# sebastian-hofstaetter/matchmaker

Hardware: NVIDIA H100
Metric: query-doc pairs scored/sec (ColBERT max-sim d=128) (higher is better)
Workload: dtype f16

## Files before the change

matchmaker_b200/build.py:

```python
from __future__ import annotations

import argparse
import hashlib
import os
import shutil
import subprocess
import sys
from concurrent.futures import ThreadPoolExecutor

HERE = os.path.dirname(os.path.abspath(__file__))
CSRC = os.path.join(HERE, "csrc")
INCLUDE = os.path.join(os.path.dirname(HERE), "include")
LIB_NAME = "libmatchmaker_b200.so"
LIB_PATH = os.path.join(CSRC, LIB_NAME)
OBJ_DIR = os.path.join(CSRC, "build")

NVCC_FLAGS = [
    "-gencode", "arch=compute_90a,code=sm_90a",
    "-O3", "-std=c++17", "-lineinfo",
    "-Xcompiler", "-fPIC",
    "-Xcompiler", "-fvisibility=hidden",
    "--expt-relaxed-constexpr",
    "-I", INCLUDE,
]


def _nvcc() -> str:
    for cand in (os.environ.get("NVCC"), shutil.which("nvcc"), "/usr/local/cuda/bin/nvcc"):
        if cand and os.path.isfile(cand):
            return cand
    raise RuntimeError("nvcc not found (set NVCC=...)")


def sources():
    return sorted(os.path.join(CSRC, f) for f in os.listdir(CSRC) if f.endswith(".cu"))


def _digest(paths) -> str:
    h = hashlib.sha256()
    for p in sorted(paths):
        h.update(p.encode())
        with open(p, "rb") as f:
            h.update(f.read())
    h.update(" ".join(NVCC_FLAGS).encode())
    return h.hexdigest()


def _all_inputs():
    hdrs = [os.path.join(CSRC, f) for f in os.listdir(CSRC) if f.endswith((".cuh", ".h"))]
    hdrs += [os.path.join(INCLUDE, f) for f in os.listdir(INCLUDE) if f.endswith(".h")]
    return sources() + hdrs


def build(force: bool = False, verbose: bool = False, prof: bool = False) -> str:
    stamp = os.path.join(OBJ_DIR, "stamp.sha256")
    digest = _digest(_all_inputs()) + ("+prof" if prof else "")
    if not force and os.path.isfile(LIB_PATH) and os.path.isfile(stamp) and open(stamp).read() == digest:
        return LIB_PATH
    os.makedirs(OBJ_DIR, exist_ok=True)
    nvcc = _nvcc()
    extra = (["-Xptxas", "-v"] if verbose else []) + (["-DMMB200_ENABLE_PROF"] if prof else [])

    def compile_one(src):
        obj = os.path.join(OBJ_DIR, os.path.basename(src)[:-3] + ".o")
        cmd = [nvcc, *NVCC_FLAGS, *extra, "-c", src, "-o", obj]
        r = subprocess.run(cmd, capture_output=True, text=True)
        if r.returncode != 0:
            raise RuntimeError(f"nvcc failed for {src}:\n{r.stdout}\n{r.stderr}")
        if verbose:
            sys.stderr.write(r.stderr)
        return obj

    with ThreadPoolExecutor(max_workers=min(8, os.cpu_count() or 1)) as ex:
        objs = list(ex.map(compile_one, sources()))
    link = [nvcc, "-shared", "-gencode", "arch=compute_90a,code=sm_90a", "-cudart", "static",
            "-Xcompiler", "-fPIC", "-o", LIB_PATH, *objs]
    r = subprocess.run(link, capture_output=True, text=True)
    if r.returncode != 0:
        raise RuntimeError(f"link failed:\n{r.stdout}\n{r.stderr}")
    with open(stamp, "w") as f:
        f.write(digest)
    return LIB_PATH


if __name__ == "__main__":
    ap = argparse.ArgumentParser()
    ap.add_argument("--force", action="store_true")
    ap.add_argument("--verbose", action="store_true")
    ap.add_argument("--prof", action="store_true", help="debugging build with the MMB200_*_PROF switches compiled in")
    a = ap.parse_args()
    print(build(force=a.force, verbose=a.verbose, prof=a.prof))
```

matchmaker_b200/csrc/maxsim_qm.cu:

```cuda
#include <cuda_bf16.h>
#include <cuda_fp16.h>

#include <algorithm>

#include "device_util.cuh"
#include "host_util.cuh"
#include "masks.cuh"
#include "maxsim.cuh"
#include "ptx.cuh"

namespace mmb {

namespace {

constexpr int kThreads = 384;
constexpr int kChunkRows = 64;
constexpr int kChunkKBlockBytes = kChunkRows * 128;
constexpr int kMaxStages = 32;
constexpr int kMaxLd = 4096;
constexpr int kScouts = 3;
constexpr int kRecordStep = 6;
constexpr int kMaxRecords = 48;
constexpr int kRecordReserve = 12 * 1024;
constexpr int kQSlots = 2;
constexpr int kQRows = 32;
constexpr int kQBlockBytes = kQRows * 128;
constexpr uint32_t kFill = 1u << 16, kLiveMask = kFill - 1;
constexpr int kRecBits = 4;
constexpr int kRegsHelper = 120, kRegsConsumer = 192;

#ifdef MMB200_ENABLE_PROF
enum QmProf {
  kPrTotal, kPrQEmpty, kPrRFull, kPrEmpty, kPrTma, kPrChunks,
  kCoTotal, kCoRFull, kCoFull, kCoIssue, kCoMma, kCoReduce, kCoEpilogue, kCoDocs,
  kScTotal, kScREmpty,
  kProfCount
};
__device__ unsigned long long g_qm_prof[kProfCount];
#define QM_PROF(...) __VA_ARGS__
#else
#define QM_PROF(...)
#endif

struct QmShared {
  uint64_t full[kMaxStages];
  uint64_t empty[kMaxStages];
  uint64_t qfull[kQSlots];
  uint64_t qempty[kQSlots];
  uint64_t rfull[kMaxRecords];
  uint64_t rempty[kMaxRecords];
  float xm[2][2][4][32];
  int32_t xa[2][2][4][32];
};

struct QmLaunch {
  int32_t kblocks;
  int32_t stages;
  int32_t chunk_bytes;
  int32_t records;
  int32_t rec_words;
};

struct RecCursor {
  int slot;
  uint32_t phase;
  __device__ __forceinline__ void advance(int step, int records) {
    slot += step;
    if (slot >= records) { slot -= records; phase ^= 1u; }
  }
};

struct QmMaps {
  CUtensorMap q;
  CUtensorMap d;
};

template <bool kStore>
struct PairStream {
  struct Batch {
    int32_t q, d, dm, rows;
    int64_t row0, row_end;
  };
  const MaxsimParams& P;
  int64_t first, end, step;
  int64_t pre_batch;
  int k;
  int lane;
  Batch cur, nxt, pre;

  __device__ __forceinline__ PairStream(const MaxsimParams& P_, int64_t first_, int64_t end_, int64_t step_, int lane_)
      : P(P_), first(first_), end(end_), step(step_), lane(lane_) {
    load1(cur, 0);
    load1(nxt, 1);
    load2(cur);
    load2(nxt);
    resolve(cur);
    pre_batch = 2;
    load1(pre, pre_batch);
    k = -1;
  }
  __device__ __forceinline__ void load1(Batch& b, int64_t bi) {
    const int64_t p = first + (bi * 32 + lane) * step;
    b.q = 0; b.d = -1; b.dm = 0; b.rows = 0; b.row0 = 0; b.row_end = 0;
    if (p >= end) return;
    b.q = P.pair_q ? P.pair_q[p] : (int32_t)((p + P.pair_base) / P.docs_per_query);
    b.d = P.pair_d ? P.pair_d[p] : (int32_t)p;
    if (P.pair_dmask) b.dm = P.pair_dmask[p];
  }
  __device__ __forceinline__ void load2(Batch& b) {
    if (!P.pair_dmask) b.dm = b.d;
    if constexpr (kStore) {
      if (b.d >= 0) { b.row0 = P.doc_offsets[b.d]; b.row_end = P.doc_offsets[b.d + 1]; }
    }
  }
  __device__ __forceinline__ void resolve(Batch& b) {
    if constexpr (kStore) b.rows = (int)max((int64_t)0, min(b.row_end - b.row0, (int64_t)P.Ld));
  }
  __device__ __forceinline__ void next() {
    if (++k == 32) {
      cur = nxt;
      resolve(cur);
      nxt = pre;
      load2(nxt);
      load1(pre, ++pre_batch);
      k = 0;
    }
  }
  __device__ __forceinline__ int64_t q() const { return __shfl_sync(0xffffffffu, cur.q, k); }
  __device__ __forceinline__ int64_t d() const { return __shfl_sync(0xffffffffu, cur.d, k); }
  __device__ __forceinline__ int64_t dm() const { return __shfl_sync(0xffffffffu, cur.dm, k); }
  __device__ __forceinline__ int rows() const { return __shfl_sync(0xffffffffu, cur.rows, k); }
  __device__ __forceinline__ int64_t row0() const { return __shfl_sync(0xffffffffu, cur.row0, k); }
};

template <typename T>
__device__ __forceinline__ void wgmma_n32(float (&d)[16], uint64_t a, uint64_t b, uint32_t acc);
template <>
__device__ __forceinline__ void wgmma_n32<__half>(float (&d)[16], uint64_t a, uint64_t b, uint32_t acc) {
  wgmma_m64n32k16_f16(d, a, b, acc);
}
template <>
__device__ __forceinline__ void wgmma_n32<__nv_bfloat16>(float (&d)[16], uint64_t a, uint64_t b, uint32_t acc) {
  wgmma_m64n32k16_bf16(d, a, b, acc);
}

template <bool kArgmax>
__device__ __forceinline__ void take(float v, int row, float& m, int& am) {
  if constexpr (kArgmax) {
    const bool gt = v > m;
    m = gt ? v : m;
    am = gt ? row : am;
  } else {
    m = fmaxf(m, v);
  }
}

template <typename T, bool kArgmax, bool kStore>
__global__ void __launch_bounds__(kThreads, 1)
maxsim_qm_kernel(const __grid_constant__ QmMaps M, MaxsimParams P, QmLaunch L) {
  extern __shared__ uint8_t smem_raw[];
  uint8_t* smem = smem_raw + ((1024u - (smem_u32(smem_raw) & 1023u)) & 1023u);
  const int qslot_bytes = L.kblocks * kQBlockBytes;
  uint8_t* q_base = smem;
  uint8_t* stage_base = q_base + kQSlots * qslot_bytes;
  uint32_t* rec_base = reinterpret_cast<uint32_t*>(stage_base + (size_t)L.stages * L.chunk_bytes);
  QmShared* S = reinterpret_cast<QmShared*>(rec_base + (size_t)L.records * L.rec_words);

  const int warp = threadIdx.x >> 5;
  const int lane = threadIdx.x & 31;

  int64_t p_begin, p_end;
  cta_share(P.n_pairs, &p_begin, &p_end);

  if (threadIdx.x == 0) {
    prefetch_tensormap(&M.q);
    prefetch_tensormap(&M.d);
    for (int s = 0; s < L.stages; ++s) { mbar_init(&S->full[s], 1); mbar_init(&S->empty[s], 4); }
    for (int s = 0; s < kQSlots; ++s) { mbar_init(&S->qfull[s], 1); mbar_init(&S->qempty[s], 8); }
    for (int r = 0; r < L.records; ++r) {
      mbar_init(&S->rfull[r], 1);
      mbar_init(&S->rempty[r], 5);
      rec_base[(size_t)r * L.rec_words + kRecBits - 2] = 0;
      rec_base[(size_t)r * L.rec_words + kRecBits - 1] = 0;
    }
    fence_barrier_init();
  }
  __syncthreads();

  if (warp == 0) {
    setmaxnreg_dec<kRegsHelper>();
    PairStream<kStore> meta(P, p_begin, p_end, 1, lane);
    const int ring = L.stages >> 1;
    int st_cur = 0, st_oth = 0;
    uint32_t ph_cur = 0, ph_oth = 0;
    int64_t prev_q = -1;
    uint32_t qcount = 0;
    RecCursor rc{0, 0};
    QM_PROF(unsigned long long prof[kProfCount] = {}; const long long t_start = clock64(); long long t_;)
    for (int64_t p = p_begin; p < p_end; ++p) {
      meta.next();
      const int64_t qi = meta.q();
      const int64_t di = meta.d();
      const int64_t row0 = kStore ? meta.row0() : 0;
      if (qi != prev_q) {
        const uint32_t slot = qcount & 1u, use = qcount >> 1;
        QM_PROF(t_ = clock64();)
        mbar_wait(&S->qempty[slot], (use & 1u) ^ 1u);
        QM_PROF(prof[kPrQEmpty] += clock64() - t_;)
        if (elect_one_sync()) {
          mbar_arrive_expect_tx(&S->qfull[slot], (uint32_t)(L.kblocks * kQBlockBytes));
          for (int kb = 0; kb < L.kblocks; ++kb)
            tma_load_4d(&M.q, q_base + (size_t)slot * qslot_bytes + kb * kQBlockBytes, &S->qfull[slot], 0, 0, kb, (int)qi,
                        kEvictLast);
        }
        __syncwarp();
        ++qcount;
        prev_q = qi;
      }
      const int c = (int)((p - p_begin) & 1);
      QM_PROF(t_ = clock64();)
      mbar_wait(&S->rfull[rc.slot], rc.phase);
      QM_PROF(prof[kPrRFull] += clock64() - t_;)
      const int live = (int)(rec_base[(size_t)rc.slot * L.rec_words] & kLiveMask);
      __syncwarp();
      if (lane == 0) mbar_arrive(&S->rempty[rc.slot]);
      rc.advance(1, L.records);
      const int dcoord = kStore ? 0 : (int)di;
      const int nch = max(1, (live + kChunkRows - 1) / kChunkRows);
      int row = kStore ? (int)row0 : live - kChunkRows * nch;
      for (int ch = 0; ch < nch; ++ch, row += kChunkRows) {
        const int stage = c * ring + st_cur;
        QM_PROF(t_ = clock64();)
        mbar_wait(&S->empty[stage], ph_cur ^ 1u);
        QM_PROF(prof[kPrEmpty] += clock64() - t_; t_ = clock64(); ++prof[kPrChunks];)
        if (elect_one_sync()) {
          if (live == 0) {
            mbar_arrive(&S->full[stage]);
          } else {
            mbar_arrive_expect_tx(&S->full[stage], (uint32_t)L.chunk_bytes);
            tma_load_4d(&M.d, stage_base + (size_t)stage * L.chunk_bytes, &S->full[stage], 0, row, 0, dcoord, kEvictFirst);
          }
        }
        __syncwarp();
        QM_PROF(prof[kPrTma] += clock64() - t_;)
        if (++st_cur == ring) { st_cur = 0; ph_cur ^= 1u; }
      }
      const int st = st_cur; st_cur = st_oth; st_oth = st;
      const uint32_t ph = ph_cur; ph_cur = ph_oth; ph_oth = ph;
    }
    QM_PROF(prof[kPrTotal] = clock64() - t_start;
            if (lane == 0) for (int i = kPrTotal; i <= kPrChunks; ++i) atomicAdd(&g_qm_prof[i], prof[i]);)
  } else if (warp <= kScouts) {
    setmaxnreg_dec<kRegsHelper>();
    constexpr int kW = 8;
    const int s = warp - 1;
    const int dmt = P.d_mask ? P.mask_dtype : MMB200_MASK_NONE;
    const int nwin = (P.Ld + 32 * kW - 1) / (32 * kW);
    const int bit_words = L.rec_words - kRecBits;
    PairStream<kStore> meta(P, p_begin + s, p_end, kScouts, lane);
    RecCursor rc{s, 0};
    int64_t fp = p_begin + s;
    auto load_win = [&](uint32_t (&raw)[kW], int64_t dm, int w) {
#pragma unroll
      for (int k = 0; k < kW; ++k) {
        const int g = w * 32 * kW + 32 * k + lane;
        raw[k] = 1;
        if (dmt != MMB200_MASK_NONE && g < P.Ld) {
          const uint64_t v = mask_raw(P.d_mask, dmt, dm * (int64_t)P.Ld + g);
          raw[k] = (uint32_t)(v | (v >> 32));
        }
      }
    };
    auto fetch = [&](uint32_t (&raw)[kW], int64_t& dm, int& lim) {
      if (fp < p_end) {
        meta.next();
        dm = meta.dm();
        lim = kStore ? meta.rows() : P.Ld;
        load_win(raw, dm, 0);
      }
      fp += kScouts;
    };
    QM_PROF(unsigned long long prof_re = 0; const long long t_start = clock64();)
    auto doc = [&](uint32_t (&raw)[kW], int64_t& dm, int& lim) {
      QM_PROF(const long long t_ = clock64();)
      mbar_wait(&S->rempty[rc.slot], rc.phase ^ 1u);
      QM_PROF(prof_re += clock64() - t_;)
      uint32_t* rec = rec_base + (size_t)rc.slot * L.rec_words;
      int live = 0;
      bool masked = false;
      for (int w = 0; w < nwin; ++w) {
        if (w > 0) load_win(raw, dm, w);
#pragma unroll
        for (int k = 0; k < kW; ++k) {
          const int g = w * 32 * kW + 32 * k + lane;
          const bool in_doc = g < lim;
          const bool ok = in_doc && mask_test(raw[k], dmt);
          masked |= in_doc && !ok;
          const uint32_t b = __ballot_sync(0xffffffffu, ok);
          const int wi = w * kW + k;
          if (b) live = 32 * wi + 32 - __clz(b);
          if (lane == 0 && wi < bit_words) rec[kRecBits + wi] = b;
        }
      }
      const bool fill = !kStore && __any_sync(0xffffffffu, masked);
      fetch(raw, dm, lim);
      if (lane == 0) {
        rec[0] = (uint32_t)live | (fill ? kFill : 0u);
        mbar_arrive(&S->rfull[rc.slot]);
      }
      rc.advance(kScouts, L.records);
    };
    uint32_t ra[kW], rb[kW];
    int64_t dma = 0, dmb = 0;
    int la = 0, lb = 0;
    fetch(ra, dma, la);
    fetch(rb, dmb, lb);
    for (int64_t sp = p_begin + s; sp < p_end;) {
      doc(ra, dma, la);
      if ((sp += kScouts) >= p_end) break;
      doc(rb, dmb, lb);
      sp += kScouts;
    }
    QM_PROF(if (lane == 0) {
      atomicAdd(&g_qm_prof[kScTotal], (unsigned long long)(clock64() - t_start));
      atomicAdd(&g_qm_prof[kScREmpty], prof_re);
    })
  } else {
    setmaxnreg_inc<kRegsConsumer>();
    const int c = (warp >> 2) - 1;
    const int wq = warp & 3;
    const int r0 = 16 * wq + (lane >> 2);
    const int qmt = P.q_mask ? P.mask_dtype : MMB200_MASK_NONE;
    const int ring = L.stages >> 1;
    int64_t prev_q = -1;
    uint32_t qcount = 0;
    int cur_slot = 0;
    RecCursor rc{c, 0};
    auto load_q = [&](int64_t n0) -> int32_t { return p_begin + n0 + lane < p_end ? P.pair_q[p_begin + n0 + lane] : 0; };
    int32_t qb_cur = 0, qb_nxt = 0;
    if (P.pair_q) { qb_cur = load_q(0); qb_nxt = load_q(32); }
    int64_t q_run = 0;
    int32_t q_rem = 0;
    if (!P.pair_q) {
      q_run = (p_begin + P.pair_base) / P.docs_per_query;
      q_rem = (int32_t)((p_begin + P.pair_base) - q_run * P.docs_per_query);
    }
    QM_PROF(unsigned long long prof[kProfCount] = {}; const long long t_start = clock64(); long long t_;)
    int64_t n_walk = 0;
    auto walk_to = [&](int64_t n) {
      for (; n_walk <= n; ++n_walk) {
        int64_t qi;
        if (P.pair_q) {
          if ((n_walk & 31) == 0 && n_walk > 0) { qb_cur = qb_nxt; qb_nxt = load_q(n_walk + 32); }
          qi = __shfl_sync(0xffffffffu, qb_cur, (int)(n_walk & 31));
        } else {
          qi = q_run;
          if (++q_rem == P.docs_per_query) { q_rem = 0; ++q_run; }
        }
        if (qi != prev_q) {
          if (prev_q >= 0) { __syncwarp(); if (lane == 0) mbar_arrive(&S->qempty[cur_slot]); }
          cur_slot = (int)(qcount & 1u);
          mbar_wait(&S->qfull[cur_slot], (qcount >> 1) & 1u);
          ++qcount;
          prev_q = qi;
        }
      }
      return prev_q;
    };
    struct Doc {
      int64_t n;
      uint32_t qlo;
      uint64_t qraw;
      int slot;
      uint32_t head;
      int live, nch;
    };
    auto begin = [&](Doc& D, int64_t n) {
      const int64_t qi = walk_to(n);
      D.n = n;
      D.qlo = (uint32_t)make_wgmma_sw128_desc(smem_u32(q_base + (size_t)cur_slot * qslot_bytes));
      D.qraw = 0;
      if (wq == 0 && lane < P.Lq)
        D.qraw = (qmt != MMB200_MASK_NONE) ? mask_raw(P.q_mask, qmt, qi * (int64_t)P.Lq + lane) : 1;
      QM_PROF(t_ = clock64();)
      mbar_wait(&S->rfull[rc.slot], rc.phase);
      QM_PROF(prof[kCoRFull] += clock64() - t_; ++prof[kCoDocs];)
      D.slot = rc.slot;
      rc.advance(2, L.records);
      D.head = rec_base[(size_t)D.slot * L.rec_words];
      D.live = (int)(D.head & kLiveMask);
      D.nch = max(1, (D.live + kChunkRows - 1) / kChunkRows);
    };
    int st_next = 0;
    uint32_t ph_next = 0;
    constexpr uint64_t kDescHi = (uint64_t)(1024 >> 4) << 32 | (uint64_t)1 << 62;
    auto issue = [&](float (&acc)[16], uint32_t qlo_doc) -> int {
      const int stage = c * ring + st_next;
      QM_PROF(t_ = clock64();)
      mbar_wait(&S->full[stage], ph_next);
      QM_PROF(prof[kCoFull] += clock64() - t_; t_ = clock64();)
      if (++st_next == ring) { st_next = 0; ph_next ^= 1u; }
      const uint32_t daddr = smem_u32(stage_base + (size_t)stage * L.chunk_bytes);
      const uint32_t dlo = (uint32_t)make_wgmma_sw128_desc(__shfl_sync(0xffffffffu, daddr, 0));
      const uint32_t qlo = __shfl_sync(0xffffffffu, qlo_doc, 0);
      wgmma_fence();
#pragma unroll
      for (int k = 0; k < 4; ++k) wgmma_n32<T>(acc, kDescHi | (dlo + 2 * k), kDescHi | (qlo + 2 * k), k != 0);
      if (L.kblocks > 1) {
#pragma unroll
        for (int k = 0; k < 4; ++k)
          wgmma_n32<T>(acc, kDescHi | (dlo + (kChunkKBlockBytes >> 4) + 2 * k),
                       kDescHi | (qlo + (kQBlockBytes >> 4) + 2 * k), 1);
      }
      wgmma_commit();
      wgmma_fence_regs(acc);
      QM_PROF(prof[kCoIssue] += clock64() - t_;)
      return stage;
    };
    float mx[8];
    int ax[8];
#pragma unroll
    for (int e = 0; e < 8; ++e) { mx[e] = -INFINITY; ax[e] = -1; }
    auto reduce = [&](float (&acc)[16], int stage, const Doc& D, int ch) {
      wgmma_fence_regs(acc);
      const int col0 = kStore ? kChunkRows * ch : D.live - kChunkRows * (D.nch - ch);
      const int x0 = col0 + r0, x1 = x0 + 8;
      const uint32_t* bits = rec_base + (size_t)D.slot * L.rec_words + kRecBits;
      const float p0 = (bits[x0 >> 5] >> (x0 & 31)) & 1u ? 0.f : -INFINITY;
      const float p1 = (bits[x1 >> 5] >> (x1 & 31)) & 1u ? 0.f : -INFINITY;
#pragma unroll
      for (int e = 0; e < 8; ++e) {
        const int i = 4 * (e >> 1) + (e & 1);
        take<kArgmax>(acc[i] + p0, x0, mx[e], ax[e]);
        take<kArgmax>(acc[i + 2] + p1, x1, mx[e], ax[e]);
      }
      __syncwarp();
      if (lane == 0) mbar_arrive(&S->empty[stage]);
    };
    auto combine = [&](float om, int oa, float& m, int& a) {
      if constexpr (kArgmax) {
        if (om > m || (om == m && (unsigned)oa < (unsigned)a)) { m = om; a = oa; }
      } else {
        m = fmaxf(m, om);
      }
    };
    auto epilogue = [&](const Doc& D) {
      QM_PROF(t_ = clock64();)
      if (lane == 0) mbar_arrive(&S->rempty[D.slot]);
#pragma unroll
      for (int o = 4; o < 32; o <<= 1) {
#pragma unroll
        for (int e = 0; e < 8; ++e) {
          const float om = __shfl_xor_sync(0xffffffffu, mx[e], o);
          const int oa = kArgmax ? __shfl_xor_sync(0xffffffffu, ax[e], o) : 0;
          combine(om, oa, mx[e], ax[e]);
        }
      }
      const int buf = (int)((D.n >> 1) & 1);
      float* xm = S->xm[c][buf][0];
      int32_t* xa = S->xa[c][buf][0];
      if (lane < 4) {
#pragma unroll
        for (int e = 0; e < 8; ++e) {
          const int t = 8 * (e >> 1) + 2 * lane + (e & 1);
          xm[32 * wq + t] = mx[e];
          if constexpr (kArgmax) xa[32 * wq + t] = ax[e];
        }
      }
#pragma unroll
      for (int e = 0; e < 8; ++e) { mx[e] = -INFINITY; ax[e] = -1; }
      if (wq != 0) {
        named_bar_arrive(1 + c, 128);
      } else {
        named_bar_sync(1 + c, 128);
        float m = xm[lane];
        int a = kArgmax ? xa[lane] : -1;
#pragma unroll
        for (int w = 1; w < 4; ++w) combine(xm[32 * w + lane], kArgmax ? xa[32 * w + lane] : 0, m, a);
        if (D.head & kFill) take<kArgmax>(-1000.f, P.Ld, m, a);
        const bool ok = mask_test(D.qraw, qmt);
        const int64_t p = p_begin + D.n;
        if constexpr (kArgmax) {
          if (lane < P.Lq) P.argmax[p * (int64_t)P.Lq + lane] = (ok && a < P.Ld) ? a : -1;
        }
        float s = ok ? m : 0.f;
        s += __shfl_down_sync(0xffffffffu, s, 8);
#pragma unroll
        for (int o = 1; o < 8; o <<= 1) s += __shfl_xor_sync(0xffffffffu, s, o);
        const float hi = __shfl_sync(0xffffffffu, s, 16);
        if (lane == 0) P.out[p] = s + hi;
      }
      QM_PROF(prof[kCoEpilogue] += clock64() - t_;)
    };
    const int64_t n_pairs = p_end - p_begin;
    float acc[16];
    for (int64_t n = c; n < n_pairs; n += 2) {
      Doc D;
      begin(D, n);
      for (int ch = 0; ch < D.nch; ++ch) {
        const int st = issue(acc, D.qlo);
        QM_PROF(t_ = clock64();)
        wgmma_wait<0>();
        QM_PROF(prof[kCoMma] += clock64() - t_; t_ = clock64();)
        reduce(acc, st, D, ch);
        QM_PROF(prof[kCoReduce] += clock64() - t_;)
      }
      epilogue(D);
    }
    QM_PROF(prof[kCoTotal] = clock64() - t_start;
            if (wq == 0 && lane == 0) for (int i = kCoTotal; i <= kCoDocs; ++i) atomicAdd(&g_qm_prof[i], prof[i]);)
  }
}

template <typename T, bool kArgmax, bool kStore>
int launch_qm(int grid, size_t smem_bytes, cudaStream_t stream, const QmMaps& M, const MaxsimParams& P,
              const QmLaunch& L) {
  MMB_CHECK_CUDA(cudaFuncSetAttribute(maxsim_qm_kernel<T, kArgmax, kStore>, cudaFuncAttributeMaxDynamicSharedMemorySize,
                                      (int)smem_bytes));
  maxsim_qm_kernel<T, kArgmax, kStore><<<grid, kThreads, smem_bytes, stream>>>(M, P, L);
  MMB_CHECK_CUDA(cudaGetLastError());
  return MMB200_OK;
}

int launch_qm_dispatch(int grid, size_t smem_bytes, cudaStream_t stream, const QmMaps& M, const MaxsimParams& P,
                       const QmLaunch& L, int dtype) {
  if (P.doc_offsets)
    return dtype == MMB200_F16 ? launch_qm<__half, false, true>(grid, smem_bytes, stream, M, P, L)
                               : launch_qm<__nv_bfloat16, false, true>(grid, smem_bytes, stream, M, P, L);
  if (dtype == MMB200_F16)
    return P.argmax ? launch_qm<__half, true, false>(grid, smem_bytes, stream, M, P, L)
                    : launch_qm<__half, false, false>(grid, smem_bytes, stream, M, P, L);
  return P.argmax ? launch_qm<__nv_bfloat16, true, false>(grid, smem_bytes, stream, M, P, L)
                  : launch_qm<__nv_bfloat16, false, false>(grid, smem_bytes, stream, M, P, L);
}

}

int maxsim_qm_launch(const MaxsimParams& P, int dtype, const DeviceInfo& dev, cudaStream_t stream, bool* handled) {
  *handled = false;
  if (dtype != MMB200_F16 && dtype != MMB200_BF16) return MMB200_OK;
  if (P.Lq > kQRows || (P.dim != 64 && P.dim != 128) || P.Ld > kMaxLd) return MMB200_OK;
  if ((reinterpret_cast<uintptr_t>(P.q) | reinterpret_cast<uintptr_t>(P.d)) & 15) return MMB200_OK;
  if (P.doc_offsets && P.argmax) return MMB200_OK;
  QmLaunch L;
  L.kblocks = P.dim / 64;
  L.chunk_bytes = L.kblocks * kChunkKBlockBytes;
  L.rec_words = kRecBits + 2 * ((P.Ld + kChunkRows - 1) / kChunkRows);
  const int fixed = kQSlots * L.kblocks * kQBlockBytes + (int)sizeof(QmShared) + 1024;
  L.stages = std::min(kMaxStages, (dev.max_smem_optin - fixed - kRecordReserve) / L.chunk_bytes) & ~1;
  const int rec_bytes = L.rec_words * 4;
  L.records = std::min(kMaxRecords, (dev.max_smem_optin - fixed - L.stages * L.chunk_bytes) / rec_bytes);
  L.records -= L.records % kRecordStep;
  if (L.stages < 4 || L.records < kRecordStep) return MMB200_OK;
  const size_t smem_bytes = (size_t)L.stages * L.chunk_bytes + (size_t)L.records * rec_bytes + fixed;

  const CUtensorMapDataType tdt = dtype == MMB200_F16 ? CU_TENSOR_MAP_DATA_TYPE_FLOAT16 : CU_TENSOR_MAP_DATA_TYPE_BFLOAT16;
  QmMaps M;
  {
    const uint64_t dims[4] = {64, (uint64_t)P.Lq, (uint64_t)L.kblocks, (uint64_t)P.n_q};
    const uint64_t strides[3] = {(uint64_t)P.dim * 2, 128, (uint64_t)P.Lq * P.dim * 2};
    const uint32_t box[4] = {64, (uint32_t)kQRows, 1, 1};
    if (int rc = encode_tensor_map(&M.q, tdt, 4, P.q, dims, strides, box, CU_TENSOR_MAP_SWIZZLE_128B,
                                   CU_TENSOR_MAP_L2_PROMOTION_L2_128B))
      return rc;
  }
  const uint64_t d_rows = P.doc_offsets ? (uint64_t)P.n_rows : (uint64_t)P.Ld;
  const uint64_t d_count = P.doc_offsets ? 1 : (uint64_t)P.n_d;
  {
    const uint64_t dims[4] = {64, d_rows, (uint64_t)L.kblocks, d_count};
    const uint64_t strides[3] = {(uint64_t)P.dim * 2, 128, d_rows * P.dim * 2};
    const uint32_t box[4] = {64, (uint32_t)kChunkRows, (uint32_t)L.kblocks, 1};
    if (int rc = encode_tensor_map(&M.d, tdt, 4, P.d, dims, strides, box, CU_TENSOR_MAP_SWIZZLE_128B,
                                   CU_TENSOR_MAP_L2_PROMOTION_L2_256B))
      return rc;
  }
  *handled = true;
  const int grid = (int)std::min<int64_t>(dev.sm_count, P.n_pairs);
#ifdef MMB200_ENABLE_PROF
  const bool prof = getenv("MMB200_MAXSIM_PROF") != nullptr;
  if (prof) {
    const unsigned long long zero[kProfCount] = {};
    MMB_CHECK_CUDA(cudaMemcpyToSymbolAsync(g_qm_prof, zero, sizeof(zero), 0, cudaMemcpyHostToDevice, stream));
  }
  const int rc = launch_qm_dispatch(grid, smem_bytes, stream, M, P, L, dtype);
  if (prof && rc == MMB200_OK) {
    unsigned long long h[kProfCount];
    MMB_CHECK_CUDA(cudaMemcpyFromSymbolAsync(h, g_qm_prof, sizeof(h), 0, cudaMemcpyDeviceToHost, stream));
    MMB_CHECK_CUDA(cudaStreamSynchronize(stream));
    const double ctas = grid, wgs = 2.0 * grid, scouts = (double)kScouts * grid;
    const double chunks = (double)h[kPrChunks], docs = (double)h[kCoDocs];
    fprintf(stderr,
            "maxsim_prof pairs %lld Ld %d chunks %.0f | cycles per CTA: producer total %.0f qempty %.0f rfull %.0f "
            "empty %.0f tma %.0f | per consumer warpgroup: total %.0f rfull %.0f full %.0f issue %.0f mma %.0f "
            "reduce %.0f epilogue %.0f | per scout: total %.0f rempty %.0f | per chunk: producer %.0f (empty %.0f, "
            "tma %.0f), warpgroup full %.0f issue %.0f mma %.0f reduce %.0f | per document per warpgroup: total %.0f "
            "epilogue %.0f rfull %.0f\n",
            (long long)P.n_pairs, P.Ld, chunks, h[kPrTotal] / ctas, h[kPrQEmpty] / ctas, h[kPrRFull] / ctas,
            h[kPrEmpty] / ctas, h[kPrTma] / ctas, h[kCoTotal] / wgs, h[kCoRFull] / wgs, h[kCoFull] / wgs,
            h[kCoIssue] / wgs, h[kCoMma] / wgs, h[kCoReduce] / wgs, h[kCoEpilogue] / wgs, h[kScTotal] / scouts,
            h[kScREmpty] / scouts, h[kPrTotal] / chunks, h[kPrEmpty] / chunks, h[kPrTma] / chunks, h[kCoFull] / chunks,
            h[kCoIssue] / chunks, h[kCoMma] / chunks, h[kCoReduce] / chunks, h[kCoTotal] / docs, h[kCoEpilogue] / docs,
            h[kCoRFull] / docs);
  }
  return rc;
#else
  return launch_qm_dispatch(grid, smem_bytes, stream, M, P, L, dtype);
#endif
}

}
```

matchmaker_b200/csrc/ptx.cuh:

```cuda
#pragma once

#include <cuda.h>
#include <cuda_runtime.h>
#include <stdint.h>

namespace mmb {

__device__ __forceinline__ uint32_t smem_u32(const void* p) {
  return static_cast<uint32_t>(__cvta_generic_to_shared(p));
}

__device__ __forceinline__ uint32_t lane_id() { return threadIdx.x & 31u; }


__device__ __forceinline__ void mbar_init(uint64_t* bar, uint32_t count) {
  asm volatile("mbarrier.init.shared::cta.b64 [%0], %1;" ::"r"(smem_u32(bar)), "r"(count) : "memory");
}

__device__ __forceinline__ void fence_barrier_init() {
  asm volatile("fence.mbarrier_init.release.cluster;" ::: "memory");
}

__device__ __forceinline__ void fence_proxy_async_smem() {
  asm volatile("fence.proxy.async.shared::cta;" ::: "memory");
}

__device__ __forceinline__ void mbar_arrive(uint64_t* bar) {
  asm volatile("{\n\t.reg .b64 st;\n\tmbarrier.arrive.shared::cta.b64 st, [%0];\n\t}" ::"r"(smem_u32(bar))
               : "memory");
}

__device__ __forceinline__ void mbar_arrive_expect_tx(uint64_t* bar, uint32_t bytes) {
  asm volatile("{\n\t.reg .b64 st;\n\tmbarrier.arrive.expect_tx.shared::cta.b64 st, [%0], %1;\n\t}" ::"r"(
                   smem_u32(bar)),
               "r"(bytes)
               : "memory");
}

#ifndef MMB_WATCHDOG_CYCLES
#define MMB_WATCHDOG_CYCLES (4000000000ll)
#endif

__device__ __forceinline__ bool mbar_try_wait(uint64_t* bar, uint32_t parity) {
  uint32_t ok;
  asm volatile(
      "{\n\t.reg .pred p;\n\t"
      "mbarrier.try_wait.parity.shared::cta.b64 p, [%1], %2;\n\t"
      "selp.u32 %0, 1, 0, p;\n\t}"
      : "=r"(ok)
      : "r"(smem_u32(bar)), "r"(parity)
      : "memory");
  return ok != 0;
}

__device__ __forceinline__ void mbar_wait(uint64_t* bar, uint32_t parity) {
  if (mbar_try_wait(bar, parity)) return;
  const long long t0 = clock64();
  while (!mbar_try_wait(bar, parity))
    if (clock64() - t0 > MMB_WATCHDOG_CYCLES) {
#ifdef MMB200_ENABLE_PROF
      printf("mmb200: mbarrier watchdog (block %d thread %d bar %u parity %u)\n", (int)blockIdx.x, (int)threadIdx.x,
             smem_u32(bar), parity);
#endif
      __trap();
    }
}

constexpr uint64_t kEvictNormal = 0x1000000000000000ull;
constexpr uint64_t kEvictFirst = 0x12F0000000000000ull;
constexpr uint64_t kEvictLast = 0x14F0000000000000ull;

__device__ __forceinline__ void prefetch_tensormap(const CUtensorMap* m) {
  asm volatile("prefetch.tensormap [%0];" ::"l"(reinterpret_cast<uint64_t>(m)) : "memory");
}

__device__ __forceinline__ void tma_load_4d(const CUtensorMap* map, void* smem_dst, uint64_t* bar, int c0,
                                            int c1, int c2, int c3, uint64_t cache_hint) {
  asm volatile(
      "cp.async.bulk.tensor.4d.shared::cluster.global.mbarrier::complete_tx::bytes.L2::cache_hint"
      " [%0], [%1, {%3, %4, %5, %6}], [%2], %7;"
      ::"r"(smem_u32(smem_dst)),
      "l"(reinterpret_cast<uint64_t>(map)), "r"(smem_u32(bar)), "r"(c0), "r"(c1), "r"(c2), "r"(c3),
      "l"(cache_hint)
      : "memory");
}

__device__ __forceinline__ void tma_load_3d(const CUtensorMap* map, void* smem_dst, uint64_t* bar, int c0,
                                            int c1, int c2, uint64_t cache_hint) {
  asm volatile(
      "cp.async.bulk.tensor.3d.shared::cluster.global.mbarrier::complete_tx::bytes.L2::cache_hint"
      " [%0], [%1, {%3, %4, %5}], [%2], %6;"
      ::"r"(smem_u32(smem_dst)),
      "l"(reinterpret_cast<uint64_t>(map)), "r"(smem_u32(bar)), "r"(c0), "r"(c1), "r"(c2), "l"(cache_hint)
      : "memory");
}

__device__ __forceinline__ void tma_load_2d(const CUtensorMap* map, void* smem_dst, uint64_t* bar, int c0,
                                            int c1, uint64_t cache_hint) {
  asm volatile(
      "cp.async.bulk.tensor.2d.shared::cluster.global.mbarrier::complete_tx::bytes.L2::cache_hint"
      " [%0], [%1, {%3, %4}], [%2], %5;"
      ::"r"(smem_u32(smem_dst)),
      "l"(reinterpret_cast<uint64_t>(map)), "r"(smem_u32(bar)), "r"(c0), "r"(c1), "l"(cache_hint)
      : "memory");
}

__device__ __forceinline__ void cp_async_16_zfill(uint32_t smem_dst, const void* gmem_src, uint32_t src_bytes) {
  asm volatile("cp.async.cg.shared.global [%0], [%1], 16, %2;" ::"r"(smem_dst), "l"(reinterpret_cast<uint64_t>(gmem_src)),
               "r"(src_bytes)
               : "memory");
}

__device__ __forceinline__ void cp_async_mbar_arrive_noinc(uint64_t* bar) {
  asm volatile("cp.async.mbarrier.arrive.noinc.shared::cta.b64 [%0];" ::"r"(smem_u32(bar)) : "memory");
}

__device__ __forceinline__ void bulk_load(void* smem_dst, const void* gmem_src, uint32_t bytes, uint64_t* bar) {
  asm volatile("cp.async.bulk.shared::cluster.global.mbarrier::complete_tx::bytes [%0], [%1], %2, [%3];"
               ::"r"(smem_u32(smem_dst)), "l"(reinterpret_cast<uint64_t>(gmem_src)), "r"(bytes), "r"(smem_u32(bar))
               : "memory");
}

__device__ __forceinline__ uint64_t make_wgmma_sw128_desc(uint32_t smem_addr) {
  uint64_t d = 0;
  d |= static_cast<uint64_t>((smem_addr & 0x3FFFFu) >> 4);
  d |= static_cast<uint64_t>(1) << 16;
  d |= static_cast<uint64_t>(1024 >> 4) << 32;
  d |= static_cast<uint64_t>(1) << 62;
  return d;
}

__device__ __forceinline__ void wgmma_fence() { asm volatile("wgmma.fence.sync.aligned;" ::: "memory"); }
__device__ __forceinline__ void wgmma_commit() { asm volatile("wgmma.commit_group.sync.aligned;" ::: "memory"); }
template <int kPending>
__device__ __forceinline__ void wgmma_wait() { asm volatile("wgmma.wait_group.sync.aligned %0;" ::"n"(kPending) : "memory"); }
template <int N>
__device__ __forceinline__ void wgmma_fence_regs(float (&d)[N]) {
#pragma unroll
  for (int i = 0; i < N; ++i) asm volatile("" : "+f"(d[i])::"memory");
}

#define MMB_ACC4(i) "+f"(d[i]), "+f"(d[i + 1]), "+f"(d[i + 2]), "+f"(d[i + 3])
#define MMB_ACC16(i) MMB_ACC4(i), MMB_ACC4(i + 4), MMB_ACC4(i + 8), MMB_ACC4(i + 12)
#define MMB_REGS16 "%0, %1, %2, %3, %4, %5, %6, %7, %8, %9, %10, %11, %12, %13, %14, %15"
#define MMB_REGS20 MMB_REGS16 ", %16, %17, %18, %19"
#define MMB_REGS32 MMB_REGS16 ", %16, %17, %18, %19, %20, %21, %22, %23, %24, %25, %26, %27, %28, %29, %30, %31"
#define MMB_REGS64                                                                                               \
  MMB_REGS32 ", %32, %33, %34, %35, %36, %37, %38, %39, %40, %41, %42, %43, %44, %45, %46, %47, "                    \
             "%48, %49, %50, %51, %52, %53, %54, %55, %56, %57, %58, %59, %60, %61, %62, %63"

#define MMB_WGMMA_SS(N, K, TY, TNSP, NR, REGS, PI, AI, BI, ...)                                                      \
  __device__ __forceinline__ void wgmma_m64n##N##k##K##_##TY(float (&d)[NR], uint64_t adesc, uint64_t bdesc,           \
                                                             uint32_t accumulate) {                                  \
    asm volatile("{\n\t.reg .pred p;\n\tsetp.ne.b32 p, " PI ", 0;\n\t"                                                 \
                 "wgmma.mma_async.sync.aligned.m64n" #N "k" #K ".f32." #TY "." #TY " {" REGS "}, " AI ", " BI          \
                 ", p, 1, 1" TNSP ";\n\t}"                                                                             \
                 : __VA_ARGS__                                                                                       \
                 : "l"(adesc), "l"(bdesc), "r"(accumulate));                                                        \
  }
MMB_WGMMA_SS(32, 16, f16, ", 0, 0", 16, MMB_REGS16, "%18", "%16", "%17", MMB_ACC16(0))
MMB_WGMMA_SS(32, 16, bf16, ", 0, 0", 16, MMB_REGS16, "%18", "%16", "%17", MMB_ACC16(0))
MMB_WGMMA_SS(64, 16, f16, ", 0, 0", 32, MMB_REGS32, "%34", "%32", "%33", MMB_ACC16(0), MMB_ACC16(16))
MMB_WGMMA_SS(64, 16, bf16, ", 0, 0", 32, MMB_REGS32, "%34", "%32", "%33", MMB_ACC16(0), MMB_ACC16(16))
MMB_WGMMA_SS(128, 16, f16, ", 0, 0", 64, MMB_REGS64, "%66", "%64", "%65", MMB_ACC16(0), MMB_ACC16(16), MMB_ACC16(32), MMB_ACC16(48))
MMB_WGMMA_SS(128, 16, bf16, ", 0, 0", 64, MMB_REGS64, "%66", "%64", "%65", MMB_ACC16(0), MMB_ACC16(16), MMB_ACC16(32), MMB_ACC16(48))
MMB_WGMMA_SS(32, 32, e4m3, "", 16, MMB_REGS16, "%18", "%16", "%17", MMB_ACC16(0))
MMB_WGMMA_SS(128, 32, e4m3, "", 64, MMB_REGS64, "%66", "%64", "%65", MMB_ACC16(0), MMB_ACC16(16), MMB_ACC16(32), MMB_ACC16(48))

#define MMB_WGMMA_RS_TF32(N, NR, REGS, A0, PI, BI, ...)                                                             \
  __device__ __forceinline__ void wgmma_m64n##N##k8_tf32_rs(float (&d)[NR], const uint32_t (&a)[4], uint64_t bdesc,     \
                                                            uint32_t accumulate) {                                   \
    asm volatile("{\n\t.reg .pred p;\n\tsetp.ne.b32 p, " PI ", 0;\n\t"                                                 \
                 "wgmma.mma_async.sync.aligned.m64n" #N "k8.f32.tf32.tf32 {" REGS "}, {" A0 "}, " BI ", p, 1, 1;\n\t}"   \
                 : __VA_ARGS__                                                                                       \
                 : "r"(a[0]), "r"(a[1]), "r"(a[2]), "r"(a[3]), "l"(bdesc), "r"(accumulate));                        \
  }
MMB_WGMMA_RS_TF32(64, 32, MMB_REGS32, "%32, %33, %34, %35", "%37", "%36", MMB_ACC16(0), MMB_ACC16(16))
MMB_WGMMA_RS_TF32(40, 20, MMB_REGS20, "%20, %21, %22, %23", "%25", "%24", MMB_ACC16(0), MMB_ACC4(16))
MMB_WGMMA_RS_TF32(32, 16, MMB_REGS16, "%16, %17, %18, %19", "%21", "%20", MMB_ACC16(0))

__device__ __forceinline__ uint32_t f32_to_tf32_rna(float x) {
  uint32_t r;
  asm("cvt.rna.tf32.f32 %0, %1;" : "=r"(r) : "f"(x));
  return r;
}

template <int kRegs>
__device__ __forceinline__ void setmaxnreg_inc() { asm volatile("setmaxnreg.inc.sync.aligned.u32 %0;" ::"n"(kRegs)); }
template <int kRegs>
__device__ __forceinline__ void setmaxnreg_dec() { asm volatile("setmaxnreg.dec.sync.aligned.u32 %0;" ::"n"(kRegs)); }

__device__ __forceinline__ uint32_t cluster_ctarank() {
  uint32_t r;
  asm volatile("mov.u32 %0, %%cluster_ctarank;" : "=r"(r));
  return r;
}
__device__ __forceinline__ void cluster_sync_all() {
  asm volatile("barrier.cluster.arrive.release.aligned;\n\tbarrier.cluster.wait.acquire.aligned;" ::: "memory");
}
__device__ __forceinline__ void tma_load_2d_multicast(const CUtensorMap* map, void* smem_dst, uint64_t* bar, int c0, int c1,
                                                      uint16_t cta_mask, uint64_t cache_hint) {
  asm volatile(
      "cp.async.bulk.tensor.2d.shared::cluster.global.mbarrier::complete_tx::bytes.multicast::cluster.L2::cache_hint"
      " [%0], [%1, {%3, %4}], [%2], %5, %6;"
      ::"r"(smem_u32(smem_dst)),
      "l"(reinterpret_cast<uint64_t>(map)), "r"(smem_u32(bar)), "r"(c0), "r"(c1), "h"(cta_mask), "l"(cache_hint)
      : "memory");
}
__device__ __forceinline__ void mbar_arrive_cluster(uint64_t* bar, uint32_t cta) {
  asm volatile(
      "{\n\t.reg .b32 ra;\n\tmapa.shared::cluster.u32 ra, %0, %1;\n\t"
      "mbarrier.arrive.release.cluster.shared::cluster.b64 _, [ra];\n\t}"
      ::"r"(smem_u32(bar)), "r"(cta)
      : "memory");
}
__device__ __forceinline__ bool elect_one_sync() {
  uint32_t pred;
  asm volatile("{\n\t.reg .pred p;\n\telect.sync _|p, 0xffffffff;\n\tselp.u32 %0, 1, 0, p;\n\t}" : "=r"(pred));
  return pred != 0;
}

__device__ __forceinline__ void named_bar_sync(uint32_t id, uint32_t nthreads) {
  asm volatile("bar.sync %0, %1;" ::"r"(id), "r"(nthreads) : "memory");
}
__device__ __forceinline__ void named_bar_arrive(uint32_t id, uint32_t nthreads) {
  asm volatile("bar.arrive %0, %1;" ::"r"(id), "r"(nthreads) : "memory");
}

__device__ __forceinline__ uint4 ldg_stream_v4(const void* p) {
  uint4 r;
  asm volatile("ld.global.nc.L1::no_allocate.v4.u32 {%0, %1, %2, %3}, [%4];"
               : "=r"(r.x), "=r"(r.y), "=r"(r.z), "=r"(r.w)
               : "l"(p));
  return r;
}

}
```

Before: 145.6 million.

## Overlap consumer epilogue with next document's first MMA and specialize mask loads

The consumer loop now begins the next document and issues its first wgmma chunk before running the previous document's epilogue, so the cross-warp reduction and output write overlap tensor-core work. The epilogue is made branch-free: all four warps sync on the named barrier and compute the reduction redundantly, with only warp 0 storing results. Scout mask loading is specialized per mask dtype with clamped indices, which removes per-element branches. The watchdog printf gets its own build flag. The gains come with more register pressure and more complex control flow in the consumer warps.

Result: faster. 149.1 million (median of 6 runs) (+2.4%).

```diff
diff --git a/matchmaker_b200/build.py b/matchmaker_b200/build.py
--- a/matchmaker_b200/build.py
+++ b/matchmaker_b200/build.py
@@ -52,14 +52,15 @@
     return sources() + hdrs
 
 
-def build(force: bool = False, verbose: bool = False, prof: bool = False) -> str:
+def build(force: bool = False, verbose: bool = False, prof: bool = False, watchdog_print: bool = False) -> str:
     stamp = os.path.join(OBJ_DIR, "stamp.sha256")
-    digest = _digest(_all_inputs()) + ("+prof" if prof else "")
+    digest = _digest(_all_inputs()) + ("+prof" if prof else "") + ("+wdprint" if watchdog_print else "")
     if not force and os.path.isfile(LIB_PATH) and os.path.isfile(stamp) and open(stamp).read() == digest:
         return LIB_PATH
     os.makedirs(OBJ_DIR, exist_ok=True)
     nvcc = _nvcc()
     extra = (["-Xptxas", "-v"] if verbose else []) + (["-DMMB200_ENABLE_PROF"] if prof else [])
+    extra += ["-DMMB200_WATCHDOG_PRINT"] if watchdog_print else []
 
     def compile_one(src):
         obj = os.path.join(OBJ_DIR, os.path.basename(src)[:-3] + ".o")
@@ -88,5 +89,6 @@
     ap.add_argument("--force", action="store_true")
     ap.add_argument("--verbose", action="store_true")
     ap.add_argument("--prof", action="store_true", help="debugging build with the MMB200_*_PROF switches compiled in")
+    ap.add_argument("--watchdog-print", action="store_true", help="debugging build whose mbarrier watchdog prints the barrier")
     a = ap.parse_args()
-    print(build(force=a.force, verbose=a.verbose, prof=a.prof))
+    print(build(force=a.force, verbose=a.verbose, prof=a.prof, watchdog_print=a.watchdog_print))
diff --git a/matchmaker_b200/csrc/maxsim_qm.cu b/matchmaker_b200/csrc/maxsim_qm.cu
--- a/matchmaker_b200/csrc/maxsim_qm.cu
+++ b/matchmaker_b200/csrc/maxsim_qm.cu
@@ -261,14 +261,28 @@
     RecCursor rc{s, 0};
     int64_t fp = p_begin + s;
     auto load_win = [&](uint32_t (&raw)[kW], int64_t dm, int w) {
-#pragma unroll
-      for (int k = 0; k < kW; ++k) {
-        const int g = w * 32 * kW + 32 * k + lane;
-        raw[k] = 1;
-        if (dmt != MMB200_MASK_NONE && g < P.Ld) {
-          const uint64_t v = mask_raw(P.d_mask, dmt, dm * (int64_t)P.Ld + g);
-          raw[k] = (uint32_t)(v | (v >> 32));
-        }
+      const int64_t row = dm * (int64_t)P.Ld;
+      auto at = [&](int k) { return row + min(w * 32 * kW + 32 * k + lane, P.Ld - 1); };
+      switch (dmt) {
+        case MMB200_MASK_U8:
+#pragma unroll
+          for (int k = 0; k < kW; ++k) raw[k] = static_cast<const uint8_t*>(P.d_mask)[at(k)];
+          break;
+        case MMB200_MASK_I32:
+        case MMB200_MASK_F32:
+#pragma unroll
+          for (int k = 0; k < kW; ++k) raw[k] = static_cast<const uint32_t*>(P.d_mask)[at(k)];
+          break;
+        case MMB200_MASK_I64:
+#pragma unroll
+          for (int k = 0; k < kW; ++k) {
+            const uint64_t v = static_cast<const uint64_t*>(P.d_mask)[at(k)];
+            raw[k] = (uint32_t)(v | (v >> 32));
+          }
+          break;
+        default:
+#pragma unroll
+          for (int k = 0; k < kW; ++k) raw[k] = 1;
       }
     };
     auto fetch = [&](uint32_t (&raw)[kW], int64_t& dm, int& lim) {
@@ -446,7 +460,6 @@
     };
     auto epilogue = [&](const Doc& D) {
       QM_PROF(t_ = clock64();)
-      if (lane == 0) mbar_arrive(&S->rempty[D.slot]);
 #pragma unroll
       for (int o = 4; o < 32; o <<= 1) {
 #pragma unroll
@@ -459,45 +472,40 @@
       const int buf = (int)((D.n >> 1) & 1);
       float* xm = S->xm[c][buf][0];
       int32_t* xa = S->xa[c][buf][0];
-      if (lane < 4) {
-#pragma unroll
-        for (int e = 0; e < 8; ++e) {
-          const int t = 8 * (e >> 1) + 2 * lane + (e & 1);
-          xm[32 * wq + t] = mx[e];
-          if constexpr (kArgmax) xa[32 * wq + t] = ax[e];
-        }
+#pragma unroll
+      for (int e = 0; e < 8; ++e) {
+        const int t = 8 * (e >> 1) + 2 * (lane & 3) + (e & 1);
+        xm[32 * wq + t] = mx[e];
+        if constexpr (kArgmax) xa[32 * wq + t] = ax[e];
       }
 #pragma unroll
       for (int e = 0; e < 8; ++e) { mx[e] = -INFINITY; ax[e] = -1; }
-      if (wq != 0) {
-        named_bar_arrive(1 + c, 128);
-      } else {
-        named_bar_sync(1 + c, 128);
-        float m = xm[lane];
-        int a = kArgmax ? xa[lane] : -1;
-#pragma unroll
-        for (int w = 1; w < 4; ++w) combine(xm[32 * w + lane], kArgmax ? xa[32 * w + lane] : 0, m, a);
-        if (D.head & kFill) take<kArgmax>(-1000.f, P.Ld, m, a);
-        const bool ok = mask_test(D.qraw, qmt);
-        const int64_t p = p_begin + D.n;
-        if constexpr (kArgmax) {
-          if (lane < P.Lq) P.argmax[p * (int64_t)P.Lq + lane] = (ok && a < P.Ld) ? a : -1;
-        }
-        float s = ok ? m : 0.f;
-        s += __shfl_down_sync(0xffffffffu, s, 8);
-#pragma unroll
-        for (int o = 1; o < 8; o <<= 1) s += __shfl_xor_sync(0xffffffffu, s, o);
-        const float hi = __shfl_sync(0xffffffffu, s, 16);
-        if (lane == 0) P.out[p] = s + hi;
-      }
+      named_bar_sync(1 + c, 128);
+      float m = xm[lane];
+      int a = kArgmax ? xa[lane] : -1;
+#pragma unroll
+      for (int w = 1; w < 4; ++w) combine(xm[32 * w + lane], kArgmax ? xa[32 * w + lane] : 0, m, a);
+      take<kArgmax>((D.head & kFill) ? -1000.f : -INFINITY, P.Ld, m, a);
+      const bool ok = mask_test(D.qraw, qmt);
+      const int64_t p = p_begin + D.n;
+      if constexpr (kArgmax) {
+        if (wq == 0 && lane < P.Lq) P.argmax[p * (int64_t)P.Lq + lane] = (ok && a < P.Ld) ? a : -1;
+      }
+      float s = ok ? m : 0.f;
+      s += __shfl_down_sync(0xffffffffu, s, 8);
+#pragma unroll
+      for (int o = 1; o < 8; o <<= 1) s += __shfl_xor_sync(0xffffffffu, s, o);
+      const float hi = __shfl_sync(0xffffffffu, s, 16);
+      if (wq == 0 && lane == 0) P.out[p] = s + hi;
       QM_PROF(prof[kCoEpilogue] += clock64() - t_;)
     };
     const int64_t n_pairs = p_end - p_begin;
     float acc[16];
+    Doc D;
+    if (c < n_pairs) begin(D, c);
+    int ch0 = 0;
     for (int64_t n = c; n < n_pairs; n += 2) {
-      Doc D;
-      begin(D, n);
-      for (int ch = 0; ch < D.nch; ++ch) {
+      for (int ch = ch0; ch < D.nch; ++ch) {
         const int st = issue(acc, D.qlo);
         QM_PROF(t_ = clock64();)
         wgmma_wait<0>();
@@ -505,7 +513,18 @@
         reduce(acc, st, D, ch);
         QM_PROF(prof[kCoReduce] += clock64() - t_;)
       }
-      epilogue(D);
+      if (lane == 0) mbar_arrive(&S->rempty[D.slot]);
+      if (n + 2 < n_pairs) {
+        const Doc done = D;
+        begin(D, n + 2);
+        const int st = issue(acc, D.qlo);
+        epilogue(done);
+        wgmma_wait<0>();
+        reduce(acc, st, D, 0);
+        ch0 = 1;
+      } else {
+        epilogue(D);
+      }
     }
     QM_PROF(prof[kCoTotal] = clock64() - t_start;
             if (wq == 0 && lane == 0) for (int i = kCoTotal; i <= kCoDocs; ++i) atomicAdd(&g_qm_prof[i], prof[i]);)
diff --git a/matchmaker_b200/csrc/ptx.cuh b/matchmaker_b200/csrc/ptx.cuh
--- a/matchmaker_b200/csrc/ptx.cuh
+++ b/matchmaker_b200/csrc/ptx.cuh
@@ -58,7 +58,7 @@
   const long long t0 = clock64();
   while (!mbar_try_wait(bar, parity))
     if (clock64() - t0 > MMB_WATCHDOG_CYCLES) {
-#ifdef MMB200_ENABLE_PROF
+#ifdef MMB200_WATCHDOG_PRINT
       printf("mmb200: mbarrier watchdog (block %d thread %d bar %u parity %u)\n", (int)blockIdx.x, (int)threadIdx.x,
              smem_u32(bar), parity);
 #endif
@@ -223,9 +223,6 @@
 __device__ __forceinline__ void named_bar_sync(uint32_t id, uint32_t nthreads) {
   asm volatile("bar.sync %0, %1;" ::"r"(id), "r"(nthreads) : "memory");
 }
-__device__ __forceinline__ void named_bar_arrive(uint32_t id, uint32_t nthreads) {
-  asm volatile("bar.arrive %0, %1;" ::"r"(id), "r"(nthreads) : "memory");
-}
 
 __device__ __forceinline__ uint4 ldg_stream_v4(const void* p) {
   uint4 r;
```
